# jedward225/MARL-HideAndSeek

Hardware: AMD Instinct MI355X
Metric: world-steps/sec (agent-steps/sec derived) at 16K worlds, 1/2/4/8 GPU (higher is better)
Workload: dtype f32; 1 GPU; 16000 worlds/GPU x 2646 steps, 2 hiders + 2 seekers, sim_flags=0, rand_seed=0, random move actions in [-5,4] each step (scripts/benchmark.py args); worlds_per_gpu=16000, total_worlds=16000, agents_per_world=4

## Files before the change

### marl-hideandseek_amd/csrc/hs_collide.h

```cpp
#pragma once
#include "hs_dev.h"

namespace hs {

enum { HULL_BOX = 0, HULL_WEDGE = 1 };

struct HullRef {
    int kind;
    V3 c, ax, ay, az, e;
};

HSD int box_face_idx(int f, int k) {
    constexpr unsigned long long t0 = (0ull) | (4ull << 3) | (6ull << 6) | (2ull << 9) |
                                      (1ull << 12) | (3ull << 15) | (7ull << 18) | (5ull << 21) |
                                      (0ull << 24) | (1ull << 27) | (5ull << 30) | (4ull << 33);
    constexpr unsigned long long t1 = (2ull) | (6ull << 3) | (7ull << 6) | (3ull << 9) |
                                      (0ull << 12) | (2ull << 15) | (3ull << 18) | (1ull << 21) |
                                      (4ull << 24) | (5ull << 27) | (7ull << 30) | (6ull << 33);
    const unsigned long long t = f < 3 ? t0 : t1;
    const int ff = f < 3 ? f : f - 3;
    return (int)((t >> (ff * 12 + k * 3)) & 7ull);
}
HSD int wedge_face_idx(int f, int k) {
    constexpr unsigned long long t = (4ull) | (1ull << 3) | (2ull << 6) | (5ull << 9) |
// ... 70 lines not shown
}
HSD V3 hull_local_vertex(int obj, int i) {
    if (obj == OBJ_RAMP) return wedge_local_v(i);
    V3 e = obj_half_extents(obj);
    return {(i & 1) ? e.x : -e.x, (i & 2) ? e.y : -e.y, (i & 4) ? e.z : -e.z};
}

HSD HullRef hull_ref_body(int obj, V3 pos, Q rot) {
    M3 m = m3_from_quat(rot);
    HullRef h;
    h.kind = obj == OBJ_RAMP ? HULL_WEDGE : HULL_BOX;
    h.c = pos; h.ax = m.c0; h.ay = m.c1; h.az = m.c2;
    h.e = obj == OBJ_RAMP ? V3{1.f, 1.f, 1.f} : obj_half_extents(obj);
    return h;
}
struct HullSrc { int kind; V3 c; Q q; V3 e; };
HSD HullSrc hull_src_body(int obj, V3 pos, Q rot) {
    return {obj == OBJ_RAMP ? HULL_WEDGE : HULL_BOX, pos, rot, obj == OBJ_RAMP ? V3{1.f, 1.f, 1.f} : obj_half_extents(obj)};
}
HSD HullSrc hull_src_wall(float cx, float cy, float hx, float hy) {
    return {HULL_BOX, V3{cx, cy, 1.25f}, Q{1.f, 0.f, 0.f, 0.f}, V3{hx, hy, 1.25f}};
}
HSD HullSrc hull_src_sel(bool c, const HullSrc &a, const HullSrc &b) {
    HullSrc r;
    r.kind = c ? a.kind : b.kind; r.c = vsel(c, a.c, b.c); r.e = vsel(c, a.e, b.e);
    r.q = {c ? a.q.w : b.q.w, c ? a.q.x : b.q.x, c ? a.q.y : b.q.y, c ? a.q.z : b.q.z};
    return r;
}
HSD HullRef hull_from(const HullSrc &s) {
    M3 m = m3_from_quat(s.q);
    HullRef h;
    h.kind = s.kind; h.c = s.c; h.ax = m.c0; h.ay = m.c1; h.az = m.c2; h.e = s.e;
    return h;
}
HSD HullRef hull_ref_wall(float cx, float cy, float hx, float hy) {
    HullRef h;
    h.kind = HULL_BOX;
    h.c = {cx, cy, 1.25f}; h.ax = {1.f, 0.f, 0.f}; h.ay = {0.f, 1.f, 0.f}; h.az = {0.f, 0.f, 1.f};
    h.e = {hx, hy, 1.25f};
    return h;
}
HSD void hull_aabb(const HullRef &h, V3 *lo_out, V3 *hi_out) {
    V3 lo = hull_v(h, 0), hi = lo;
    const int nv = hull_nv(h);
#pragma unroll
    for (int i = 1; i < 8; ++i) {
        if (i < nv) {
            V3 p = hull_v(h, i);
            lo = {fminf(lo.x, p.x), fminf(lo.y, p.y), fminf(lo.z, p.z)};
            hi = {fmaxf(hi.x, p.x), fmaxf(hi.y, p.y), fmaxf(hi.z, p.z)};
        }
    }
    *lo_out = lo; *hi_out = hi;
}

struct RawManifold { V3 n; int np; V3 pA[4]; V3 pB[4]; int vidx[4]; };

HSD float box_radius(const HullRef &h, V3 n) {
    return hs_fma(fabsf(dot(n, h.az)), h.e.z, hs_fma(fabsf(dot(n, h.ay)), h.e.y, fabsf(dot(n, h.ax)) * h.e.x));
}
struct WedgeVerts { V3 v[6]; };
HSD void wedge_verts(const HullRef &h, WedgeVerts &wv) {
#pragma unroll
    for (int i = 0; i < 6; ++i) wv.v[i] = hull_v(h, i);
}
HSD float support_min(const HullRef &h, const WedgeVerts &wv, V3 n) {
// ... 68 lines not shown
            for (int k = 1; k < 4; ++k) if (depth[k] < depth[mi]) mi = k;
            if (!(dep > depth[mi])) continue;
            slot = mi;
        }
#pragma unroll
        for (int k = 0; k < 4; ++k)
            if (k == slot) { depth[k] = dep; vi = (vi & ~(7 << (3 * k))) | (i << (3 * k)); }
    }
    *idx = vi;
    return np;
}

HSD void closest_seg_seg(V3 p1, V3 q1, V3 p2, V3 q2, V3 *c1, V3 *c2) {
    V3 d1 = q1 - p1, d2 = q2 - p2, r = p1 - p2;
    float a = dot(d1, d1), e = dot(d2, d2), f = dot(d2, r);
    float c = dot(d1, r), b = dot(d1, d2);
    float denom = a * e - b * b;
    float s = 0.f, t;
    if (denom > 1e-9f) { s = (b * f - c * e) / denom; s = fminf(fmaxf(s, 0.f), 1.f); }
    t = (b * s + f) / e;
    if (t < 0.f) { t = 0.f; s = fminf(fmaxf(-c / a, 0.f), 1.f); }
    else if (t > 1.f) { t = 1.f; s = fminf(fmaxf((b - c) / a, 0.f), 1.f); }
    *c1 = p1 + d1 * s; *c2 = p2 + d2 * t;
}

constexpr int kSatPairs = 32;
constexpr int kClipLanes = 48;
constexpr int clip_words(int lanes) { return 2 * 8 * 3 * lanes; }
struct ClipBuf { float *base; int lane; int stride; };
HSD V3 cb_get(const ClipBuf &b, int w, int i) {
    const float *p = b.base + ((w * 8 + i) * 3) * b.stride + b.lane;
    return {p[0], p[b.stride], p[2 * b.stride]};
}
HSD void cb_set(const ClipBuf &b, int w, int i, V3 v) {
    float *p = b.base + ((w * 8 + i) * 3) * b.stride + b.lane;
    p[0] = v.x; p[b.stride] = v.y; p[2 * b.stride] = v.z;
}

HSD int clip_face_contact(const HullRef &R, int fr, V3 nr, const HullRef &I, const ClipBuf &cb, V3 *pInc, float *dist_out) {
    const float dr = hull_fd(R, fr, nr);
    const int inf = hull_nf(I);
    int fi = 0; float best = dot(nr, hull_fn(I, 0));
    for (int f = 1; f < inf; ++f) { float d = dot(nr, hull_fn(I, f)); if (d < best) { best = d; fi = f; } }
    int n = hull_fcnt(I, fi);
    int cur_buf = 0;
    for (int k = 0; k < n; ++k) cb_set(cb, 0, k, hull_v(I, hull_fidx(I, fi, k)));
    const int rc = hull_fcnt(R, fr);
    for (int k = 0; k < rc && n > 0; ++k) {
        const int k1 = (k + 1 == rc) ? 0 : k + 1;
        V3 v0 = hull_v(R, hull_fidx(R, fr, k)), v1 = hull_v(R, hull_fidx(R, fr, k1));
        V3 s = cross(v1 - v0, nr);
        int m = 0;
        const int src = cur_buf, dst = cur_buf ^ 1;
        V3 prev = cb_get(cb, src, n - 1); float dprev = dot(s, prev - v0);
        for (int i = 0; i < n; ++i) {
            V3 cur = cb_get(cb, src, i); float dcur = dot(s, cur - v0);
            bool in_prev = dprev <= 0.f, in_cur = dcur <= 0.f;
            if (in_prev != in_cur) {
                float t = dprev / (dprev - dcur);
                if (m < 8) { cb_set(cb, dst, m, madd(prev, cur - prev, t)); m++; }
            }
            if (in_cur) { if (m < 8) { cb_set(cb, dst, m, cur); m++; } }
            prev = cur; dprev = dcur;
        }
        n = m;
        cur_buf = dst;
    }
    const int src = cur_buf, pts = cur_buf ^ 1;
    int c = 0;
    for (int i = 0; i < n; ++i) {
        V3 p = cb_get(cb, src, i);
        float d = dot(nr, p) - dr;
        if (d <= 0.f) { cb_set(cb, pts, c, p); c++; }
    }
#define HS_PT(i) cb_get(cb, pts, (i))
#define HS_DIST(i) (dot(nr, HS_PT(i)) - dr)
    if (c <= 4) {
#pragma unroll
        for (int i = 0; i < 4; ++i) if (i < c) { pInc[i] = HS_PT(i); dist_out[i] = HS_DIST(i); }
        return c;
    }
    int i0 = 0; float d0 = HS_DIST(0);
    for (int i = 1; i < c; ++i) { float d = HS_DIST(i); if (d < d0) { d0 = d; i0 = i; } }
    const V3 p0 = HS_PT(i0);
    int i1 = -1; float bd = -1.f;
    for (int i = 0; i < c; ++i) { if (i == i0) continue; float d2 = len2(HS_PT(i) - p0); if (d2 > bd) { bd = d2; i1 = i; } }
    const V3 p1 = HS_PT(i1);
    int i2 = -1, i3 = -1; float amax = 0.f, amin = 0.f;
    for (int i = 0; i < c; ++i) {
        if (i == i0 || i == i1) continue;
        V3 p = HS_PT(i);
        float ar = dot(cross(p0 - p, p1 - p), nr);
        if (i2 < 0 || ar > amax) { amax = ar; i2 = i; }
    }
    for (int i = 0; i < c; ++i) {
        if (i == i0 || i == i1 || i == i2) continue;
        V3 p = HS_PT(i);
        float ar = dot(cross(p0 - p, p1 - p), nr);
        if (i3 < 0 || ar < amin) { amin = ar; i3 = i; }
    }
    pInc[0] = p0; dist_out[0] = HS_DIST(i0);
    pInc[1] = p1; dist_out[1] = HS_DIST(i1);
    pInc[2] = HS_PT(i2); dist_out[2] = HS_DIST(i2);
    pInc[3] = HS_PT(i3); dist_out[3] = HS_DIST(i3);
#undef HS_PT
#undef HS_DIST
    return 4;
}

struct AxisResult { int code; V3 ax; };
HSD int pair_swap(int x) { return __builtin_amdgcn_update_dpp(0, x, 0xB1, 0xF, 0xF, false); }
HSD float pair_swap(float x) { return __int_as_float(pair_swap(__float_as_int(x))); }
HSD AxisResult sat_axes(const HullSrc &sa, const HullSrc &sb, const bool hi) {
    AxisResult res = {0, {0.f, 0.f, 0.f}};
    float bestA, bestB; int fa, fb;
    {
        const HullRef X = hull_from(hull_src_sel(hi, sb, sa)), Y = hull_from(hull_src_sel(hi, sa, sb));
        WedgeVerts wx = {}, wy = {};
        if (X.kind == HULL_WEDGE) wedge_verts(X, wx);
        if (Y.kind == HULL_WEDGE) wedge_verts(Y, wy);
        float best = 0.f; int fx = -1; int sep = 0;
        const int xnf = hull_nf(X);
        for (int f = 0; f < xnf; ++f) {
            V3 fn = hull_fn(X, f);
            float s = support_min(Y, wy, fn) - hull_fd_w(X, wx, f, fn);
            if (s > 0.f) { sep = 1; break; }
            if (fx < 0 || s > best) { best = s; fx = f; }
        }
        const float best_o = pair_swap(best); const int fx_o = pair_swap(fx);
        if (sep | pair_swap(sep)) return res;
        bestA = hi ? best_o : best; fa = hi ? fx_o : fx;
        bestB = hi ? best : best_o; fb = hi ? fx : fx_o;
    }
    const HullRef A = hull_from(sa), B = hull_from(sb);
    WedgeVerts wa = {}, wb = {};
    if (A.kind == HULL_WEDGE) wedge_verts(A, wa);
    if (B.kind == HULL_WEDGE) wedge_verts(B, wb);
    float bestE = 0.f; int ea = -1, eb = -1; V3 axE = {0.f, 0.f, 0.f};
    {
        V3 ab = B.c - A.c;
        const int aned = hull_ned(A), bned = hull_ned(B);
        const int tot = aned * bned, p0 = hi ? tot / 2 : 0, p1 = hi ? tot : tot / 2;
        int sep = 0;
        for (int p = p0; p < p1; ++p) {
            const int i = p / bned, j = p - i * bned;
            V3 ax = cross(hull_ed(A, i), hull_ed(B, j));
            float l2 = len2(ax);
            if (l2 < 1e-6f) continue;
            ax = ax * (1.f / sqrtf(l2));
            if (dot(ax, ab) < 0.f) ax = -ax;
            float s = support_min(B, wb, ax) - support_max(A, wa, ax);
            if (s > 0.f) { sep = 1; break; }
            if (ea < 0 || s > bestE) { bestE = s; ea = i; eb = j; axE = ax; }
        }
        if (sep | pair_swap(sep)) return res;
        const float bE_o = pair_swap(bestE); const int ea_o = pair_swap(ea), eb_o = pair_swap(eb);
        const V3 ax_o = {pair_swap(axE.x), pair_swap(axE.y), pair_swap(axE.z)};
        if (hi) return res;
        if (ea_o >= 0 && (ea < 0 || bE_o > bestE)) { bestE = bE_o; ea = ea_o; eb = eb_o; axE = ax_o; }
    }
    const float bestF = fmaxf(bestA, bestB);
    if (ea >= 0 && bestE > 0.9f * bestF + 0.0025f) { res.code = 1 | (ea << 4) | (eb << 8); res.ax = axE; return res; }
    const bool refB = bestB > 0.98f * bestA + 0.00125f;
    res.code = 2 | ((refB ? fb : fa) << 4) | ((refB ? 1 : 0) << 8);
    return res;
}

// ... 114 lines not shown
```

### marl-hideandseek_amd/csrc/hs_k_physics.h

```cpp
#pragma once
#include "hs_state.h"
#include "hs_rays.h"
#include "hs_collide.h"
#include "hs_solver.h"
#include "hs_broadphase.h"
#include "hs_solve_order.h"
#include "hs_k_reset.h"

namespace hs {

constexpr int kPhysThreads = 64;
constexpr int kWorldLanes = kPhysThreads / kTile;
constexpr int kLdsWalls = 32;
static_assert(kMaxSCand <= 32 && kMaxDDCand <= 16, "accepted-manifold masks are one word per world");
constexpr int kAllDD = kNumDSlots * (kNumDSlots - 1) / 2;
constexpr int kAllSC = kNumDSlots * (kMaxWalls + kMaxPlanes - 1);
constexpr int kSpInfoWords = kNumDSlots + 1;

struct alignas(16) OctRes {
    static constexpr int kClip = kClipLanes;
    static constexpr int kClipWords = clip_words(kClip);
    static constexpr int kSatPairs = kClip < hs::kSatPairs ? kClip : hs::kSatPairs;
    static constexpr int kMaxItems = kTile * (kMaxDDCand + kMaxSCand);
    static constexpr int kSlots = kClip < 31 ? kClip : 31;
// ... 446 lines not shown
    if (l == 0) {
        R.spill[g] = (unsigned char)((spillDD ? 1 : 0) | (spillSC ? 2 : 0));
        if (spillDD || spillSC) spInfo[0] = tot_dd | (tot_sc << 16);
        R.ndd[g] = (unsigned char)min(tot_dd, kMaxDDCand); R.nsc[g] = (unsigned char)min(tot_sc, kMaxSCand);
        if (R.wid[g] >= 0 && tot_dd + tot_sc > 0) S.loadAcc[R.wid[g]] += tot_dd + tot_sc;
    }
    wave_sync();
    return ic;
}

template <bool POS, int UNROLL, typename SetLam>
HSD void static_manifold(BodyS &me, const ManS &m, SetLam set_lam) {
    BodyS none;
    body_refresh_inertia(me);
    const V3 n = ld3(m.n);
    const int np = m.np;
    const float mu = POS ? m.muS : m.muD;
#pragma unroll UNROLL
    for (int j = 0; j < 4; ++j)
        if (j < np) {
            const float lamj = m.lam[j];
            if (POS) set_lam(j, lamj + solve_point_position<false>(me, none, n, ld3(m.rA[j]), V3{0.f, 0.f, 0.f}, m.offB[j], mu));
            else solve_point_velocity<false>(me, none, n, ld3(m.rA[j]), V3{0.f, 0.f, 0.f}, lamj, mu);
        }
}

#define HS_COLD __device__ __forceinline__
struct SpillCtx {
    const float *walls, *planes;
    ManDD *wsDD; ManS *wsSC; unsigned short *spPair; int *spInfo;
    int wbeg;
};
HSD SpillCtx spill_ctx(const SimState &S) { return {S.walls.p, S.planes.p, (ManDD *)S.wsDD, (ManS *)S.wsSC, S.spPair, S.spInfo, S.wbeg}; }
HSD HullSrc sat_hull_b(const Col<float, 4 * kMaxWalls> &walls, const OctRes &R, int g, int w, bool isdd, int bsel);

HS_COLD void spill_sat(SpillCtx c, OctRes *Rp) {
    OctRes &R = *Rp;
    const int lane = hs_lane() & 63;
    const bool hi = (lane & 1) != 0;
    const Col<float, 4 * kMaxWalls> walls = {const_cast<float *>(c.walls)};
    const Col<float, 4 * kMaxPlanes> planes = {const_cast<float *>(c.planes)};
#pragma unroll 1
    for (int g = 0; g < kTile; ++g) {
        const int fl = __builtin_amdgcn_readfirstlane((int)R.spill[g]);
        if (fl == 0) continue;
        const int w = c.wbeg + g;
        const int tot = __builtin_amdgcn_readfirstlane(c.spInfo[(size_t)w * kSpInfoWords]);
#pragma unroll 1
        for (int kind = 0; kind < 2; ++kind) {
            if ((fl & (1 << kind)) == 0) continue;
            const bool isdd = kind == 0;
            const int n = isdd ? tot & 0xffff : tot >> 16;
#pragma unroll 1
            for (int base = isdd ? kMaxDDCand : kMaxSCand; base < n; base += OctRes::kSatPairs) {
                const int kk = base + (lane >> 1);
                if (kk < n && (lane >> 1) < OctRes::kSatPairs) {
                    const int pair = c.spPair[(size_t)w * (kAllDD + kAllSC) + (isdd ? 0 : kAllDD) + kk];
                    const int a = pair_a(pair), bsel = pair_b(pair);
                    const int oa = meta_obj(R.meta[a][g]);
                    const V3 pa = rld3(R.pos, a, g);
                    const Q qa = rld4(R.rot, a, g);
                    ManDD *const md = c.wsDD + (size_t)w * kAllDD + kk;
                    ManS *const ms = c.wsSC + (size_t)w * kAllSC + kk;
                    RawManifold raw;
                    raw.np = 0;
                    bool plane = false;
                    if (!isdd && bsel >= kMaxWalls) {
// ... 70 lines not shown
                if (POS) { rbody_store_pose(R, g, ba, Ab); rbody_store_pose(R, g, bb, Bb); }
                else { rbody_store_vel(R, g, ba, Ab); rbody_store_vel(R, g, bb, Bb); }
                wave_sync();
            }
        }
    }
}

template <bool POS>
HS_COLD void spill_static(SpillCtx c, OctRes *Rp, int NS) {
    OctRes &R = *Rp;
#pragma unroll 1
    for (int g = 0; g < kTile; ++g) {
        if ((__builtin_amdgcn_readfirstlane((int)R.spill[g]) & 2) == 0) continue;
        const int w = c.wbeg + g;
        const int slot = hs_lane();
        if (slot >= NS) continue;
        const int info = c.spInfo[(size_t)w * kSpInfoWords + 1 + slot];
        const int first = info & 0xffff, cnt = info >> 16;
        if (cnt == 0) continue;
        BodyS me;
        rbody_load(R, g, slot, me);
#pragma unroll 1
        for (int k = first; k < first + cnt; ++k) {
            ManS &m = c.wsSC[(size_t)w * kAllSC + k];
            if (m.np <= 0) continue;
            static_manifold<POS, 1>(me, m, [&](int j, float v) { m.lam[j] = v; });
        }
        if (POS) rbody_store_pose(R, g, slot, me); else rbody_store_vel(R, g, slot, me);
    }
}

HSD HullSrc sat_hull_a(const OctRes &R, int g, int a) { return hull_src_body(meta_obj(R.meta[a][g]), rld3(R.pos, a, g), rld4(R.rot, a, g)); }
HSD HullSrc sat_hull_b(const Col<float, 4 * kMaxWalls> &walls, const OctRes &R, int g, int w, bool isdd, int bsel) {
    static_assert(kNumDSlots <= kMaxWalls, "a body slot is a valid wall row");
    const float *const wp = &walls(min(bsel, kMaxWalls - 1), w);
    const float cx = glb_word(wp), cy = glb_word(wp + kMaxWalls * kTile);
    const float hx = glb_word(wp + 2 * kMaxWalls * kTile), hy = glb_word(wp + 3 * kMaxWalls * kTile);
    const int slot = isdd ? bsel : 0;
    const HullSrc body = hull_src_body(meta_obj(R.meta[slot][g]), rld3(R.pos, slot, g), rld4(R.rot, slot, g));
    return hull_src_sel(isdd, body, hull_src_wall(cx, cy, hx, hy));
}
HSD bool sat_flush(const SimState &S, OctRes &R, int npend, bool last) {
    const int lane = hs_lane() & 63;
    const bool toLds = last && lane < OctRes::kSlots;
    bool wroteGlobal = false;
    int mw[kManWords]; int mkind = 0, mkk = 0, mg = 0, mpair = 0;
    if (lane < npend) {
        const int item = R.u.sat.pend[0][lane] & 0xffff;
        AxisResult res;
        res.code = R.u.sat.pend[0][lane] >> 16;
        res.ax = {__int_as_float(R.u.sat.pend[1][lane]), __int_as_float(R.u.sat.pend[2][lane]), __int_as_float(R.u.sat.pend[3][lane])};
        const int g = item >> 6, idx = item & 63;
        const int w = S.wbeg + g;
        const bool isdd = idx < 32;
        const int kk = idx & 31;
        const int pair = isdd ? R.ddPair[kk][g] : R.scPair[kk][g];
        const int a = pair_a(pair), bsel = pair_b(pair);
        const ClipBuf cb = {R.u.sat.clip, lane, OctRes::kClip};
        RawManifold raw;
        const bool plane = res.code == 3;
        bool have;
        if (plane) {
            const int p = bsel - kMaxWalls;
            const V3 pn = {S.planes(0 * kMaxPlanes + p, w), S.planes(1 * kMaxPlanes + p, w), S.planes(2 * kMaxPlanes + p, w)};
            have = collide_hull_plane(hull_ref_body(meta_obj(R.meta[a][g]), rld3(R.pos, a, g), rld4(R.rot, a, g)), pn, S.planes(3 * kMaxPlanes + p, w), raw);
        } else {
            have = sat_contact(sat_hull_a(R, g, a), sat_hull_b(S.walls, R, g, w, isdd, bsel), res, cb, raw);
        }
        if (have) {
            const int oa = meta_obj(R.meta[a][g]);
            const int ob = isdd ? meta_obj(R.meta[bsel][g]) : plane ? OBJ_PLANE : OBJ_WALL;
            const V3 pa = rld3(R.pos, a, g);
            const Q qai = qinv(rld4(R.rot, a, g));
            const float muS = 0.5f * (obj_mu_s(oa) + obj_mu_s(ob)), muD = 0.5f * (obj_mu_d(oa) + obj_mu_d(ob));
            if (isdd) {
                ManDD m;
                m.a = a; m.b = bsel; m.np = raw.np; m.muS = muS; m.muD = muD;
                st3(m.n, raw.n);
                const V3 pb = rld3(R.pos, bsel, g);
                const Q qbi = qinv(rld4(R.rot, bsel, g));
#pragma unroll
                for (int j = 0; j < 4; ++j) {
                    const bool on = j < raw.np;
                    st3(m.rA[j], on ? qrot(qai, raw.pA[j] - pa) : V3{0.f, 0.f, 0.f});
                    st3(m.rB[j], on ? qrot(qbi, raw.pB[j] - pb) : V3{0.f, 0.f, 0.f});
                    m.lam[j] = 0.f;
                }
                if (toLds) { __builtin_memcpy(mw, &m, sizeof(m)); mkind = 1; mkk = kk; mg = g; mpair = pair; }
                else { ((ManDD *)S.wsDD + (size_t)w * kAllDD)[kk] = m; wroteGlobal = true; }
                atomicOr(&R.ddAcc[g], 1u << kk);
            } else {
                ManS m;
                m.np = raw.np; m.muS = muS; m.muD = muD; m.pad[0] = 0.f; m.pad[1] = 0.f;
                st3(m.n, raw.n);
#pragma unroll
                for (int j = 0; j < 4; ++j) {
                    const bool on = j < raw.np;
                    st3(m.rA[j], !on ? V3{0.f, 0.f, 0.f} : plane ? hull_local_vertex(oa, raw.vidx[j]) : qrot(qai, raw.pA[j] - pa));
                    m.offB[j] = on ? dot(raw.pB[j], raw.n) : 0.f; m.lam[j] = 0.f;
                }
                if (toLds) { __builtin_memcpy(mw, &m, sizeof(m)); mkind = 2; mkk = kk; mg = g; mpair = pair; }
                else { ((ManS *)S.wsSC + (size_t)w * kAllSC)[kk] = m; wroteGlobal = true; }
                atomicOr(&R.scAcc[g], 1u << kk);
            }
        }
    }
    wave_sync(); __builtin_amdgcn_wave_barrier();
    if (mkind != 0) {
        int4 *dst = reinterpret_cast<int4 *>(R.u.sat.clip + lane * kManWords);
#pragma unroll
        for (int k = 0; k < (int)(sizeof(ManS) / 16); ++k) dst[k] = int4{mw[4 * k], mw[4 * k + 1], mw[4 * k + 2], mw[4 * k + 3]};
        if (mkind == 1) {
#pragma unroll
// ... 268 lines not shown
    if (__builtin_expect(anySpill, 0)) { spill_dd<POS>(spill_ctx(S), &R); wave_sync(); }
    return ord;
}

struct WallLists { int nwb, nEarly; };
template <int ROUNDS>
HSD WallLists list_wall_bodies(OctRes &R, int nbodies, int lastRound) {
    const int L = hs_lane();
    int n = 0, nEarly = 0;
#pragma unroll
    for (int r = 0; r < ROUNDS; ++r) {
        if (r == lastRound) nEarly = n;
        const bool valid = r * 64 + L < nbodies;
        const int t = valid ? R.bodies[r * 64 + L] : 0;
        const int sci = valid ? R.scInfo[t >> 3][t & 7] : 0;
        const bool on = sci != 0 && ((R.scAcc[t & 7] >> (sci & 0xff)) & ((1u << (sci >> 8)) - 1u)) != 0u;
        const unsigned long long m = __ballot(on);
        if (on) { R.wallBodies[n + __popcll(m & ((1ull << L) - 1ull))] = (unsigned char)t; atomicOr(&R.wallSeen[t & 7], 1u << (t >> 3)); }
        n += __popcll(m);
    }
    wave_sync();
    return {n, nEarly};
}

HSD void ground_pos(OctRes &R, BodyReg &b, int slot, int g, int meta) {
    if (meta_resp(meta) != RESP_DYNAMIC || b.np == 0) return;
    const int obj = meta_obj(meta);
    BodyS me;
    rbody_load(R, g, slot, me);
    const V3 gn = -V3{R.plane0[0][g], R.plane0[1][g], R.plane0[2][g]};
    const float gmuS = 0.5f * (obj_mu_s(obj) + obj_mu_s(OBJ_PLANE));
    const bool yaw = slot >= kAgentSlot0;
    float dj[4] = {0.f, 0.f, 0.f, 0.f}, share = 0.f;
    if (yaw) share = yaw_ground_prepass(me, gn, b.np, hull_local_vertex(obj, b.vidx & 7), hull_local_vertex(obj, (b.vidx >> 3) & 7),
                                        hull_local_vertex(obj, (b.vidx >> 6) & 7), hull_local_vertex(obj, (b.vidx >> 9) & 7), kGroundOff, dj);
#pragma unroll
    for (int j = 0; j < 4; ++j)
        if (j < b.np) b.lam[j] += solve_point_position_ground(me, gn, hull_local_vertex(obj, (b.vidx >> (3 * j)) & 7), kGroundOff, gmuS,
                                                              yaw, dj[j], share);
    rbody_store_pose(R, g, slot, me);
}
HSD void ground_vel(OctRes &R, const BodyReg &b, int slot, int g, int meta) {
    if (meta_resp(meta) != RESP_DYNAMIC || b.np == 0) return;
    const int obj = meta_obj(meta);
    BodyS me, none;
    rbody_load(R, g, slot, me);
    const V3 gn = -V3{R.plane0[0][g], R.plane0[1][g], R.plane0[2][g]};
    const float gmuD = 0.5f * (obj_mu_d(obj) + obj_mu_d(OBJ_PLANE));
#pragma unroll
    for (int j = 0; j < 4; ++j)
        if (j < b.np) solve_point_velocity<false>(me, none, gn, hull_local_vertex(obj, (b.vidx >> (3 * j)) & 7), V3{0.f, 0.f, 0.f},
                                                  b.lam[j], gmuD);
    rbody_store_vel(R, g, slot, me);
}
template <bool POS>
HSD void wall_round(const SimState &S, OctRes &R, int first, int nwb) {
    for (int i = first + hs_lane(); i < nwb; i += 64) {
        const int t = R.wallBodies[i];
        const int slot = t >> 3, g = t & 7;
        const int sci = R.scInfo[slot][g];
        const int bsc = sci & 0xff, asc = sci >> 8;
        const unsigned acc = R.scAcc[g];
        ManS *const wsSC = (ManS *)S.wsSC + (size_t)(S.wbeg + g) * kAllSC;
        BodyS me;
        rbody_load(R, g, slot, me);
        unsigned todo = (acc >> bsc) & ((1u << asc) - 1u);
#pragma unroll 1
        while (todo != 0u) {
            const int k = bsc + __ffs((int)todo) - 1;
            todo &= todo - 1u;
            const int loc = pair_loc(R.scPair[k][g]);
            ManS m;
// ... 12 lines not shown
    unsigned todo = 0u; int bsc = 0;
    if (walls) {
        const int t = R.wallBodies[mi];
        slot = t >> 3; g = t & 7; meta = R.meta[slot][g];
        const int sci = R.scInfo[slot][g];
        bsc = sci & 0xff;
        todo = (R.scAcc[g] >> bsc) & ((1u << (sci >> 8)) - 1u);
    } else if (valid && meta_resp(meta) == RESP_DYNAMIC && b.np != 0) {
        todo = 1u;
    }
    if (todo == 0u) return;
    const int obj = meta_obj(meta);
    BodyS me, none;
    rbody_load(R, g, slot, me);
    ManS *const wsSC = (ManS *)S.wsSC + (size_t)(S.wbeg + g) * kAllSC;
#pragma unroll 1
    while (todo != 0u) {
        const int k = bsc + __ffs((int)todo) - 1;
        todo &= todo - 1u;
        V3 n; float mu; int np, loc = kLocGlobal;
        ManS m;
        if (walls) {
            loc = pair_loc(R.scPair[k][g]);
            man_static_load(R.u.sat.clip, loc, wsSC + k, m);
            n = ld3(m.n); mu = POS ? m.muS : m.muD; np = m.np;
        } else {
            n = -V3{R.plane0[0][g], R.plane0[1][g], R.plane0[2][g]};
            mu = POS ? 0.5f * (obj_mu_s(obj) + obj_mu_s(OBJ_PLANE)) : 0.5f * (obj_mu_d(obj) + obj_mu_d(OBJ_PLANE));
            np = b.np;
        }
        body_refresh_inertia(me);
        const bool yaw = POS && !walls && slot >= kAgentSlot0;
        float dj[4] = {0.f, 0.f, 0.f, 0.f}, share = 0.f;
        if (yaw) share = yaw_ground_prepass(me, n, np, hull_local_vertex(obj, b.vidx & 7), hull_local_vertex(obj, (b.vidx >> 3) & 7),
                                            hull_local_vertex(obj, (b.vidx >> 6) & 7), hull_local_vertex(obj, (b.vidx >> 9) & 7), kGroundOff, dj);
#define HS_LAST_POINT(j)                                                                                                   \
        if ((j) < np) {                                                                                                    \
            const V3 rAj = walls ? ld3(m.rA[j]) : hull_local_vertex(obj, (b.vidx >> (3 * (j))) & 7);                       \
            const float lamj = walls ? m.lam[j] : b.lam[j];                                                                \
            if (POS) {                                                                                                     \
                const float nl = lamj + solve_point_position_ground(me, n, rAj, walls ? m.offB[j] : kGroundOff, mu, yaw, dj[j], share); \
                if (!walls) b.lam[j] = nl; else m.lam[j] = nl;                                                             \
            } else {                                                                                                       \
                solve_point_velocity<false>(me, none, n, rAj, V3{0.f, 0.f, 0.f}, lamj, mu);                                \
            }                                                                                                              \
        }
        HS_LAST_POINT(0) HS_LAST_POINT(1) HS_LAST_POINT(2) HS_LAST_POINT(3)
#undef HS_LAST_POINT
        if (POS && walls) man_put_lam(R.u.sat.clip, loc, wsSC + k, Piece{m.lam[0], m.lam[1], m.lam[2], m.lam[3]});
    }
    if (POS) rbody_store_pose(R, g, slot, me); else rbody_store_vel(R, g, slot, me);
}
HSD void derive_body_velocity(OctRes &R, int slot, int g, int meta) {
    if (meta_resp(meta) != RESP_DYNAMIC) return;
    BodyS me;
    me.pos = rld3(R.pos, slot, g); me.rot = rld4(R.rot, slot, g);
    me.ppos = rld3(R.ppos, slot, g); me.prot = rld4(R.prot, slot, g);
    derive_velocity(me);
    rbody_store_vel(R, g, slot, me);
}

HSD void action_system(const SimState &S, OctRes &R, int g, int A_, int teams) {
    const int w = S.wbeg + g;
    const ResGeom geom = {R, S, g, w};
    for (int i = 0; i < A_; ++i) {
        const int fl = R.actGL[i][g];
        if (fl == 0) continue;
        const int type = team_agent_type(teams, i);
        const int slot = kAgentSlot0 + i;
        const V3 mpos = geom.g_pos(slot);
        const Q mrot = geom.g_rot(slot);
        if (fl & 2) {
            float t; V3 o = mpos + V3{0.f, 0.f, 0.5f};
            int hit = trace_ray(geom, o, qrot(mrot, {0.f, 1.f, 0.f}), 2.5f, &t);
            if (hit >= 0 && hit < kNumDSlots) {
                const int m = R.meta[hit][g];
                const int obj = meta_obj(m), resp = meta_resp(m), owner = meta_owner(m);
// ... 356 lines not shown
```

### marl-hideandseek_amd/csrc/hs_solver.h

```cpp
#pragma once
#include "hs_state.h"
#include "hs_rays.h"
#include "hs_collide.h"

namespace hs {

struct alignas(16) ManDD { int a, b, np; float muS, muD; float n[3]; float rA[4][3]; float rB[4][3]; float lam[4]; };
struct alignas(16) ManS { int np; float muS, muD; float n[3]; float pad[2]; float rA[4][3]; float offB[4]; float lam[4]; };
static_assert(sizeof(ManDD) == 144 && sizeof(ManS) == 112, "manifold layout");

HSD bool has_mass_i(float invM, V3 invI) { return invM != 0.f || invI.z != 0.f || invI.x != 0.f || invI.y != 0.f; }

struct BodyS { V3 pos; Q rot; V3 ppos; Q prot; V3 lin, ang; float invM; V3 invI; Sym3 Iw; };

HSD void body_refresh_inertia(BodyS &b) {
    b.Iw = has_mass_i(b.invM, b.invI) ? world_inv_inertia(b.rot, b.invI) : Sym3{0.f, 0.f, 0.f, 0.f, 0.f, 0.f};
}

HSD V3 ld3(const float *p) { return {p[0], p[1], p[2]}; }
HSD Q ld4(const float *p) { return {p[0], p[1], p[2], p[3]}; }
HSD void st3(float *p, V3 v) { p[0] = v.x; p[1] = v.y; p[2] = v.z; }
HSD void st4(float *p, Q q) { p[0] = q.w; p[1] = q.x; p[2] = q.y; p[3] = q.z; }

HSD V3 apply_inv_inertia(const BodyS &b, V3 v) { return sym_mul(b.Iw, v); }
// ... 35 lines not shown
    float excess = dprev - kMaxDepenVel * kSubstepH;
    if (excess > 0.f) d = d - excess;
    if (!(d > 0.f)) return 0.f;
    float wA = gen_inv_mass(A, rAw, n);
    float wB = HAS_B ? gen_inv_mass(B, rBw, n) : 0.f;
    float wsum = wA + wB;
    if (!(wsum > 0.f)) return 0.f;
    float lam = d / wsum;
    apply_pos_impulse<HAS_B>(A, rAw, B, rBw, n * lam);
    rAw = qrot(A.rot, rAl);
    pA = A.pos + rAw;
    V3 dp;
    if (HAS_B) {
        rBw = qrot(B.rot, rBl);
        pB = B.pos + rBw;
        dp = (pA - pAprev) - (pB - pBprev);
    } else {
        dp = pA - pAprev;
    }
    V3 dpt = nmadd(dp, n, dot(dp, n));
    float lt2 = len2(dpt);
    if (lt2 > 1e-12f) {
        float wtA = gen_inv_mass_sq(A, rAw, dpt, lt2);
        float wtB = HAS_B ? gen_inv_mass_sq(B, rBw, dpt, lt2) : 0.f;
        float wts = wtA + wtB;
        if (wts > 0.f) {
            float lim = (muS * lam) * wts;
            if ((lt2 * lt2) * lt2 < lim * lim) apply_pos_impulse<HAS_B>(A, rAw, B, rBw, dpt * (lt2 / wts));
        }
    }
    return lam;
}

HSD float solve_point_position_ground(BodyS &A, V3 n, V3 rAl, float offB, float muS, bool yaw, float dj, float share) {
    BodyS none;
    V3 rAw = qrot(A.rot, rAl);
    V3 pA = A.pos + rAw;
    const V3 pAprev = A.ppos + qrot(A.prot, rAl);
    float lam;
    if (!yaw) {
        float d = dot_add(pA, n, -offB);
        if (!(d > 0.f)) return 0.f;
        const float dprev = dot_add(pAprev, n, -offB);
        const float excess = dprev - kMaxDepenVel * kSubstepH;
        if (excess > 0.f) d = d - excess;
        if (!(d > 0.f)) return 0.f;
        const float wsum = gen_inv_mass(A, rAw, n);
        if (!(wsum > 0.f)) return 0.f;
        lam = d / wsum;
        apply_pos_impulse<false>(A, rAw, none, V3{0.f, 0.f, 0.f}, n * lam);
        rAw = qrot(A.rot, rAl);
        pA = A.pos + rAw;
    } else {
        if (!(dj > 0.f)) return 0.f;
        lam = share;
    }
    const V3 dp = pA - pAprev;
    const V3 dpt = nmadd(dp, n, dot(dp, n));
    const float lt2 = len2(dpt);
    if (lt2 > 1e-12f) {
        const float wts = gen_inv_mass_sq(A, rAw, dpt, lt2);
        if (wts > 0.f) {
            const float lim = (muS * lam) * wts;
            if ((lt2 * lt2) * lt2 < lim * lim) apply_pos_impulse<false>(A, rAw, none, V3{0.f, 0.f, 0.f}, dpt * (lt2 / wts));
        }
    }
    return lam;
}
HSD float yaw_ground_prepass(BodyS &A, V3 n, int np, V3 r0, V3 r1, V3 r2, V3 r3, float off, float (&dj)[4]) {
    int k = 0; float dmax = 0.f;
#pragma unroll
    for (int j = 0; j < 4; ++j) {
        dj[j] = 0.f;
        if (j < np) {
            const V3 r = j == 0 ? r0 : j == 1 ? r1 : j == 2 ? r2 : r3;
            float d = dot_add(A.pos + qrot(A.rot, r), n, -off);
            if (d > 0.f) {
                const float excess = dot_add(A.ppos + qrot(A.prot, r), n, -off) - kMaxDepenVel * kSubstepH;
                if (excess > 0.f) d = d - excess;
            }
            dj[j] = d;
            if (d > 0.f) { k++; dmax = fmaxf(dmax, d); }
        }
    }
    if (k == 0 || !(A.invM > 0.f)) {
#pragma unroll
        for (int j = 0; j < 4; ++j) dj[j] = 0.f;
        return 0.f;
    }
    const float lamT = dmax / A.invM;
    A.pos = nmadd(A.pos, n * lamT, A.invM);
    return lamT / (float)k;
}

template <bool HAS_B>
HSD void solve_point_velocity(BodyS &A, BodyS &B, V3 n, V3 rAl, V3 rBl, float lamN, float muD) {
    if (!(lamN > 0.f)) return;
    V3 rAw = qrot(A.rot, rAl);
    V3 rBw = HAS_B ? qrot(B.rot, rBl) : V3{0.f, 0.f, 0.f};
    V3 v = {0.f, 0.f, 0.f};
    if (A.invM + A.invI.x + A.invI.y + A.invI.z != 0.f) v = cross_add(A.ang, rAw, A.lin);
    if (HAS_B && B.invM + B.invI.x + B.invI.y + B.invI.z != 0.f) v = v - cross_add(B.ang, rBw, B.lin);
    float vn = dot(n, v);
    V3 vt = nmadd(v, n, vn);
    float vt2 = len2(vt);
    V3 dv = -(n * vn);
    if (vt2 > 1e-18f) {
        float vtl = sqrtf(vt2);
        float mag = fminf((muD * lamN) * kInvSubstepH, vtl);
        dv = nmadd(dv, vt, mag / vtl);
    }
// ... 17 lines not shown
```

Measured before the change: 35.70 million world-steps/s.

## Eliminate redundant recomputation in contact clipping, SAT, and ground solver

Several small redundancy removals. Clip vertex loop reuses the previous edge endpoint, contact distances are cached in the clip buffer, and the two min/max area passes are merged into one. SAT reuses the already-built hull refs instead of rebuilding them, and sat_flush loads body meta/pose once. The ground solver precomputes each contact's previous-frame point once and shares it between the yaw prepass and the position solve. The cost is more live registers and some added conditional logic.

```diff
diff --git a/marl-hideandseek_amd/csrc/hs_collide.h b/marl-hideandseek_amd/csrc/hs_collide.h
--- a/marl-hideandseek_amd/csrc/hs_collide.h
+++ b/marl-hideandseek_amd/csrc/hs_collide.h
@@ -126,6 +126,12 @@
     HullRef h;
     h.kind = s.kind; h.c = s.c; h.ax = m.c0; h.ay = m.c1; h.az = m.c2; h.e = s.e;
     return h;
+}
+HSD HullRef hull_ref_sel(bool c, const HullRef &a, const HullRef &b) {
+    HullRef r;
+    r.kind = c ? a.kind : b.kind; r.c = vsel(c, a.c, b.c); r.e = vsel(c, a.e, b.e);
+    r.ax = vsel(c, a.ax, b.ax); r.ay = vsel(c, a.ay, b.ay); r.az = vsel(c, a.az, b.az);
+    return r;
 }
 HSD HullRef hull_ref_wall(float cx, float cy, float hx, float hy) {
     HullRef h;
@@ -260,6 +266,8 @@
     const float *p = b.base + ((w * 8 + i) * 3) * b.stride + b.lane;
     return {p[0], p[b.stride], p[2 * b.stride]};
 }
+HSD float cb_get_x(const ClipBuf &b, int w, int i) { return b.base[((w * 8 + i) * 3) * b.stride + b.lane]; }
+HSD void cb_set_x(const ClipBuf &b, int w, int i, float x) { b.base[((w * 8 + i) * 3) * b.stride + b.lane] = x; }
 HSD void cb_set(const ClipBuf &b, int w, int i, V3 v) {
     float *p = b.base + ((w * 8 + i) * 3) * b.stride + b.lane;
     p[0] = v.x; p[b.stride] = v.y; p[2 * b.stride] = v.z;
@@ -274,9 +282,14 @@
     int cur_buf = 0;
     for (int k = 0; k < n; ++k) cb_set(cb, 0, k, hull_v(I, hull_fidx(I, fi, k)));
     const int rc = hull_fcnt(R, fr);
+    const V3 vfirst = hull_v(R, hull_fidx(R, fr, 0));
+    V3 vnext = vfirst;
     for (int k = 0; k < rc && n > 0; ++k) {
         const int k1 = (k + 1 == rc) ? 0 : k + 1;
-        V3 v0 = hull_v(R, hull_fidx(R, fr, k)), v1 = hull_v(R, hull_fidx(R, fr, k1));
+        const V3 v0 = vnext;
+        V3 v1 = vfirst;
+        if (k1 != 0) v1 = hull_v(R, hull_fidx(R, fr, k1));
+        vnext = v1;
         V3 s = cross(v1 - v0, nr);
         int m = 0;
         const int src = cur_buf, dst = cur_buf ^ 1;
@@ -299,10 +312,10 @@
     for (int i = 0; i < n; ++i) {
         V3 p = cb_get(cb, src, i);
         float d = dot(nr, p) - dr;
-        if (d <= 0.f) { cb_set(cb, pts, c, p); c++; }
+        if (d <= 0.f) { cb_set(cb, pts, c, p); cb_set_x(cb, src, c, d); c++; }
     }
 #define HS_PT(i) cb_get(cb, pts, (i))
-#define HS_DIST(i) (dot(nr, HS_PT(i)) - dr)
+#define HS_DIST(i) cb_get_x(cb, src, (i))
     if (c <= 4) {
 #pragma unroll
         for (int i = 0; i < 4; ++i) if (i < c) { pInc[i] = HS_PT(i); dist_out[i] = HS_DIST(i); }
@@ -314,20 +327,17 @@
     int i1 = -1; float bd = -1.f;
     for (int i = 0; i < c; ++i) { if (i == i0) continue; float d2 = len2(HS_PT(i) - p0); if (d2 > bd) { bd = d2; i1 = i; } }
     const V3 p1 = HS_PT(i1);
-    int i2 = -1, i3 = -1; float amax = 0.f, amin = 0.f;
+    int i2 = -1, m1 = -1, m2 = -1; float amax = 0.f, a1 = 0.f, a2 = 0.f;
     for (int i = 0; i < c; ++i) {
         if (i == i0 || i == i1) continue;
         V3 p = HS_PT(i);
         float ar = dot(cross(p0 - p, p1 - p), nr);
         if (i2 < 0 || ar > amax) { amax = ar; i2 = i; }
-    }
-    for (int i = 0; i < c; ++i) {
-        if (i == i0 || i == i1 || i == i2) continue;
-        V3 p = HS_PT(i);
-        float ar = dot(cross(p0 - p, p1 - p), nr);
-        if (i3 < 0 || ar < amin) { amin = ar; i3 = i; }
-    }
-    pInc[0] = p0; dist_out[0] = HS_DIST(i0);
+        if (m1 < 0 || ar < a1) { a2 = a1; m2 = m1; a1 = ar; m1 = i; }
+        else if (m2 < 0 || ar < a2) { a2 = ar; m2 = i; }
+    }
+    const int i3 = m1 != i2 ? m1 : m2;
+    pInc[0] = p0; dist_out[0] = d0;
     pInc[1] = p1; dist_out[1] = HS_DIST(i1);
     pInc[2] = HS_PT(i2); dist_out[2] = HS_DIST(i2);
     pInc[3] = HS_PT(i3); dist_out[3] = HS_DIST(i3);
@@ -342,8 +352,8 @@
 HSD AxisResult sat_axes(const HullSrc &sa, const HullSrc &sb, const bool hi) {
     AxisResult res = {0, {0.f, 0.f, 0.f}};
     float bestA, bestB; int fa, fb;
+    const HullRef X = hull_from(hull_src_sel(hi, sb, sa)), Y = hull_from(hull_src_sel(hi, sa, sb));
     {
-        const HullRef X = hull_from(hull_src_sel(hi, sb, sa)), Y = hull_from(hull_src_sel(hi, sa, sb));
         WedgeVerts wx = {}, wy = {};
         if (X.kind == HULL_WEDGE) wedge_verts(X, wx);
         if (Y.kind == HULL_WEDGE) wedge_verts(Y, wy);
@@ -360,7 +370,7 @@
         bestA = hi ? best_o : best; fa = hi ? fx_o : fx;
         bestB = hi ? best : best_o; fb = hi ? fx : fx_o;
     }
-    const HullRef A = hull_from(sa), B = hull_from(sb);
+    const HullRef A = hull_ref_sel(hi, Y, X), B = hull_ref_sel(hi, X, Y);
     WedgeVerts wa = {}, wb = {};
     if (A.kind == HULL_WEDGE) wedge_verts(A, wa);
     if (B.kind == HULL_WEDGE) wedge_verts(B, wb);
diff --git a/marl-hideandseek_amd/csrc/hs_k_physics.h b/marl-hideandseek_amd/csrc/hs_k_physics.h
--- a/marl-hideandseek_amd/csrc/hs_k_physics.h
+++ b/marl-hideandseek_amd/csrc/hs_k_physics.h
@@ -502,7 +502,7 @@
     int wbeg;
 };
 HSD SpillCtx spill_ctx(const SimState &S) { return {S.walls.p, S.planes.p, (ManDD *)S.wsDD, (ManS *)S.wsSC, S.spPair, S.spInfo, S.wbeg}; }
-HSD HullSrc sat_hull_b(const Col<float, 4 * kMaxWalls> &walls, const OctRes &R, int g, int w, bool isdd, int bsel);
+HSD HullSrc sat_hull_b(const Col<float, 4 * kMaxWalls> &walls, const OctRes &R, int g, int w, bool isdd, int bsel, int *objB = nullptr);
 
 HS_COLD void spill_sat(SpillCtx c, OctRes *Rp) {
     OctRes &R = *Rp;
@@ -639,13 +639,15 @@
 }
 
 HSD HullSrc sat_hull_a(const OctRes &R, int g, int a) { return hull_src_body(meta_obj(R.meta[a][g]), rld3(R.pos, a, g), rld4(R.rot, a, g)); }
-HSD HullSrc sat_hull_b(const Col<float, 4 * kMaxWalls> &walls, const OctRes &R, int g, int w, bool isdd, int bsel) {
+HSD HullSrc sat_hull_b(const Col<float, 4 * kMaxWalls> &walls, const OctRes &R, int g, int w, bool isdd, int bsel, int *objB) {
     static_assert(kNumDSlots <= kMaxWalls, "a body slot is a valid wall row");
     const float *const wp = &walls(min(bsel, kMaxWalls - 1), w);
     const float cx = glb_word(wp), cy = glb_word(wp + kMaxWalls * kTile);
     const float hx = glb_word(wp + 2 * kMaxWalls * kTile), hy = glb_word(wp + 3 * kMaxWalls * kTile);
     const int slot = isdd ? bsel : 0;
-    const HullSrc body = hull_src_body(meta_obj(R.meta[slot][g]), rld3(R.pos, slot, g), rld4(R.rot, slot, g));
+    const int obj = meta_obj(R.meta[slot][g]);
+    if (objB) *objB = obj;
+    const HullSrc body = hull_src_body(obj, rld3(R.pos, slot, g), rld4(R.rot, slot, g));
     return hull_src_sel(isdd, body, hull_src_wall(cx, cy, hx, hy));
 }
 HSD bool sat_flush(const SimState &S, OctRes &R, int npend, bool last) {
@@ -668,25 +670,29 @@
         RawManifold raw;
         const bool plane = res.code == 3;
         bool have;
+        const int oa = meta_obj(R.meta[a][g]);
+        const V3 pa = rld3(R.pos, a, g);
+        const Q qa = rld4(R.rot, a, g);
+        int obB = OBJ_NONE;
+        HullSrc hb = hull_src_body(oa, pa, qa);
         if (plane) {
             const int p = bsel - kMaxWalls;
             const V3 pn = {S.planes(0 * kMaxPlanes + p, w), S.planes(1 * kMaxPlanes + p, w), S.planes(2 * kMaxPlanes + p, w)};
-            have = collide_hull_plane(hull_ref_body(meta_obj(R.meta[a][g]), rld3(R.pos, a, g), rld4(R.rot, a, g)), pn, S.planes(3 * kMaxPlanes + p, w), raw);
+            have = collide_hull_plane(hull_ref_body(oa, pa, qa), pn, S.planes(3 * kMaxPlanes + p, w), raw);
         } else {
-            have = sat_contact(sat_hull_a(R, g, a), sat_hull_b(S.walls, R, g, w, isdd, bsel), res, cb, raw);
+            hb = sat_hull_b(S.walls, R, g, w, isdd, bsel, &obB);
+            have = sat_contact(hull_src_body(oa, pa, qa), hb, res, cb, raw);
         }
         if (have) {
-            const int oa = meta_obj(R.meta[a][g]);
-            const int ob = isdd ? meta_obj(R.meta[bsel][g]) : plane ? OBJ_PLANE : OBJ_WALL;
-            const V3 pa = rld3(R.pos, a, g);
-            const Q qai = qinv(rld4(R.rot, a, g));
+            const int ob = isdd ? obB : plane ? OBJ_PLANE : OBJ_WALL;
+            const Q qai = qinv(qa);
             const float muS = 0.5f * (obj_mu_s(oa) + obj_mu_s(ob)), muD = 0.5f * (obj_mu_d(oa) + obj_mu_d(ob));
             if (isdd) {
                 ManDD m;
                 m.a = a; m.b = bsel; m.np = raw.np; m.muS = muS; m.muD = muD;
                 st3(m.n, raw.n);
-                const V3 pb = rld3(R.pos, bsel, g);
-                const Q qbi = qinv(rld4(R.rot, bsel, g));
+                const V3 pb = hb.c;
+                const Q qbi = qinv(hb.q);
 #pragma unroll
                 for (int j = 0; j < 4; ++j) {
                     const bool on = j < raw.np;
@@ -1021,12 +1027,18 @@
     const float gmuS = 0.5f * (obj_mu_s(obj) + obj_mu_s(OBJ_PLANE));
     const bool yaw = slot >= kAgentSlot0;
     float dj[4] = {0.f, 0.f, 0.f, 0.f}, share = 0.f;
-    if (yaw) share = yaw_ground_prepass(me, gn, b.np, hull_local_vertex(obj, b.vidx & 7), hull_local_vertex(obj, (b.vidx >> 3) & 7),
-                                        hull_local_vertex(obj, (b.vidx >> 6) & 7), hull_local_vertex(obj, (b.vidx >> 9) & 7), kGroundOff, dj);
-#pragma unroll
-    for (int j = 0; j < 4; ++j)
-        if (j < b.np) b.lam[j] += solve_point_position_ground(me, gn, hull_local_vertex(obj, (b.vidx >> (3 * j)) & 7), kGroundOff, gmuS,
-                                                              yaw, dj[j], share);
+    const V3 r0 = hull_local_vertex(obj, b.vidx & 7), r1 = hull_local_vertex(obj, (b.vidx >> 3) & 7);
+    const V3 r2 = hull_local_vertex(obj, (b.vidx >> 6) & 7), r3 = hull_local_vertex(obj, (b.vidx >> 9) & 7);
+    V3 q0 = {0.f, 0.f, 0.f}, q1 = q0, q2 = q0, q3 = q0;
+    q0 = prev_point(me, r0);
+    if (b.np > 1) q1 = prev_point(me, r1);
+    if (b.np > 2) q2 = prev_point(me, r2);
+    if (b.np > 3) q3 = prev_point(me, r3);
+    if (yaw) share = yaw_ground_prepass(me, gn, b.np, r0, r1, r2, r3, q0, q1, q2, q3, kGroundOff, dj);
+    b.lam[0] += solve_point_position_ground(me, gn, r0, q0, kGroundOff, gmuS, yaw, dj[0], share);
+    if (b.np > 1) b.lam[1] += solve_point_position_ground(me, gn, r1, q1, kGroundOff, gmuS, yaw, dj[1], share);
+    if (b.np > 2) b.lam[2] += solve_point_position_ground(me, gn, r2, q2, kGroundOff, gmuS, yaw, dj[2], share);
+    if (b.np > 3) b.lam[3] += solve_point_position_ground(me, gn, r3, q3, kGroundOff, gmuS, yaw, dj[3], share);
     rbody_store_pose(R, g, slot, me);
 }
 HSD void ground_vel(OctRes &R, const BodyReg &b, int slot, int g, int meta) {
@@ -1105,17 +1117,25 @@
         body_refresh_inertia(me);
         const bool yaw = POS && !walls && slot >= kAgentSlot0;
         float dj[4] = {0.f, 0.f, 0.f, 0.f}, share = 0.f;
-        if (yaw) share = yaw_ground_prepass(me, n, np, hull_local_vertex(obj, b.vidx & 7), hull_local_vertex(obj, (b.vidx >> 3) & 7),
-                                            hull_local_vertex(obj, (b.vidx >> 6) & 7), hull_local_vertex(obj, (b.vidx >> 9) & 7), kGroundOff, dj);
+#define HS_LAST_ARM(j) (walls ? ld3(m.rA[j]) : hull_local_vertex(obj, (b.vidx >> (3 * (j))) & 7))
+        const V3 rA0 = HS_LAST_ARM(0), rA1 = HS_LAST_ARM(1), rA2 = HS_LAST_ARM(2), rA3 = HS_LAST_ARM(3);
+#undef HS_LAST_ARM
+        V3 pv0 = {0.f, 0.f, 0.f}, pv1 = pv0, pv2 = pv0, pv3 = pv0;
+        if (POS) {
+            if (0 < np) pv0 = prev_point(me, rA0);
+            if (1 < np) pv1 = prev_point(me, rA1);
+            if (2 < np) pv2 = prev_point(me, rA2);
+            if (3 < np) pv3 = prev_point(me, rA3);
+        }
+        if (yaw) share = yaw_ground_prepass(me, n, np, rA0, rA1, rA2, rA3, pv0, pv1, pv2, pv3, kGroundOff, dj);
 #define HS_LAST_POINT(j)                                                                                                   \
         if ((j) < np) {                                                                                                    \
-            const V3 rAj = walls ? ld3(m.rA[j]) : hull_local_vertex(obj, (b.vidx >> (3 * (j))) & 7);                       \
             const float lamj = walls ? m.lam[j] : b.lam[j];                                                                \
             if (POS) {                                                                                                     \
-                const float nl = lamj + solve_point_position_ground(me, n, rAj, walls ? m.offB[j] : kGroundOff, mu, yaw, dj[j], share); \
+                const float nl = lamj + solve_point_position_ground(me, n, rA##j, pv##j, walls ? m.offB[j] : kGroundOff, mu, yaw, dj[j], share); \
                 if (!walls) b.lam[j] = nl; else m.lam[j] = nl;                                                             \
             } else {                                                                                                       \
-                solve_point_velocity<false>(me, none, n, rAj, V3{0.f, 0.f, 0.f}, lamj, mu);                                \
+                solve_point_velocity<false>(me, none, n, rA##j, V3{0.f, 0.f, 0.f}, lamj, mu);                              \
             }                                                                                                              \
         }
         HS_LAST_POINT(0) HS_LAST_POINT(1) HS_LAST_POINT(2) HS_LAST_POINT(3)
diff --git a/marl-hideandseek_amd/csrc/hs_solver.h b/marl-hideandseek_amd/csrc/hs_solver.h
--- a/marl-hideandseek_amd/csrc/hs_solver.h
+++ b/marl-hideandseek_amd/csrc/hs_solver.h
@@ -91,11 +91,11 @@
     return lam;
 }
 
-HSD float solve_point_position_ground(BodyS &A, V3 n, V3 rAl, float offB, float muS, bool yaw, float dj, float share) {
+HSD V3 prev_point(const BodyS &A, V3 rAl) { return A.ppos + qrot(A.prot, rAl); }
+HSD float solve_point_position_ground(BodyS &A, V3 n, V3 rAl, V3 pAprev, float offB, float muS, bool yaw, float dj, float share) {
     BodyS none;
     V3 rAw = qrot(A.rot, rAl);
     V3 pA = A.pos + rAw;
-    const V3 pAprev = A.ppos + qrot(A.prot, rAl);
     float lam;
     if (!yaw) {
         float d = dot_add(pA, n, -offB);
@@ -126,7 +126,7 @@
     }
     return lam;
 }
-HSD float yaw_ground_prepass(BodyS &A, V3 n, int np, V3 r0, V3 r1, V3 r2, V3 r3, float off, float (&dj)[4]) {
+HSD float yaw_ground_prepass(BodyS &A, V3 n, int np, V3 r0, V3 r1, V3 r2, V3 r3, V3 q0, V3 q1, V3 q2, V3 q3, float off, float (&dj)[4]) {
     int k = 0; float dmax = 0.f;
 #pragma unroll
     for (int j = 0; j < 4; ++j) {
@@ -135,7 +135,7 @@
             const V3 r = j == 0 ? r0 : j == 1 ? r1 : j == 2 ? r2 : r3;
             float d = dot_add(A.pos + qrot(A.rot, r), n, -off);
             if (d > 0.f) {
-                const float excess = dot_add(A.ppos + qrot(A.prot, r), n, -off) - kMaxDepenVel * kSubstepH;
+                const float excess = dot_add(j == 0 ? q0 : j == 1 ? q1 : j == 2 ? q2 : q3, n, -off) - kMaxDepenVel * kSubstepH;
                 if (excess > 0.f) d = d - excess;
             }
             dj[j] = d;
```

Result: faster. 36.26 million world-steps/s, median of 6 (+1.6%).
